# shuoshuof/Humanoid-Real-Time-Retarget

Measured on AMD Instinct MI355X. Metric: retargeted frames/sec + max joint-angle err vs ref, Hu humanoid @1/2/4/8 GPU, higher is better.
Workload: dtype f32; 1 GPU; VtrdynFullBodyPosRetargeter batched solve, Hu v5 target (BASELINE config 3); global_batch=262144, parallelism=dp1, input_layout=soa, input_ring_sets=3, precise_gripper=True, launch=K plain launches, step i on stream i % 2

## Files before the change

__graft_entry__.py:

```python
from __future__ import annotations

import os
import shutil
import subprocess
import sys

REPO = os.path.dirname(os.path.abspath(__file__))
PKG = os.path.join(REPO, "humanoid-real-time-retarget_amd")
ORACLE = os.path.join(REPO, "oracle")
for _p in (PKG, ORACLE):
    if _p not in sys.path:
        sys.path.insert(0, _p)


def _jobs() -> str:
    return str(min(16, os.cpu_count() or 1))


CSRC = os.path.join(PKG, "csrc")
FASTMATH_SRC = os.path.join(REPO, "tools", "check_fastmath.hip")
FASTMATH_BIN = os.path.join(REPO, "tools", "check_fastmath")
FDIV_SRC = os.path.join(REPO, "tools", "check_fdiv.hip")
FDIV_BIN = os.path.join(REPO, "tools", "check_fdiv")
FETCH_CALIB_BIN = os.path.join(REPO, "tools", "fetch_calib")


def _make(*args, env=None) -> None:
    env = dict(os.environ if env is None else env)
    env.setdefault("HIPCC", shutil.which("hipcc") or "/opt/rocm/bin/hipcc")
    subprocess.run(["make", "-C", CSRC, *args], check=True, env=env)


def build_fastmath_check(env=None) -> str:
    _make("check_fastmath", env=env)
    return FASTMATH_BIN


def build_fdiv_check(env=None) -> str:
    _make("check_fdiv", env=env)
    return FDIV_BIN


def build_fetch_calib(env=None) -> str:
    _make("fetch_calib", env=env)
    return FETCH_CALIB_BIN


def build() -> None:
    env = dict(os.environ)
    env.setdefault("HIPCC", shutil.which("hipcc") or "/opt/rocm/bin/hipcc")
    _make("-j", _jobs(), "all", "variants", env=env)
    subprocess.run(["make", "-C", ORACLE], check=True, env=env)
    build_fastmath_check(env)
    build_fdiv_check(env)
    build_fetch_calib(env)
    from rtg.build_ext import build_frame_post
    build_frame_post()
    import rtg
    from rtg import _lib
    _lib.lib()


def smoke() -> None:
    import numpy as np
    import torch

    import oracle as orc
    from rtg import _lib, assets
    from rtg.runtime import Solver

    assert torch.cuda.is_available(), "smoke() needs a HIP device"
    g = np.load(os.path.join(REPO, "tests", "golden", "full_body_pos_precise.npz"))
    zp = np.load(os.path.join(REPO, "tests", "golden", "zero_pose.npz"))
    n = 256
    body, lh, rh = (np.ascontiguousarray(g[k][:n]) for k in ("body", "lh", "rh"))
    S = Solver(_lib.SOLVER_FULL_BODY_POS, zp["vtrdyn_full_local_t"], zp["vtrdyn_full_global_t"],
               assets.parents("vtrdyn_full"), precise_gripper=True)
    dof, _, _ = S.retarget([torch.from_numpy(a).cuda() for a in (body, lh, rh)])
    torch.cuda.synchronize()
    dof = dof.cpu().numpy()
    odof, _, _ = orc.full_body_pos(zp["vtrdyn_full_local_t"], zp["vtrdyn_full_global_t"], body, lh, rh, True,
                                   want_rot=False)
    diff_oracle = float(np.abs(dof - odof).max())
    diff_ref = float(np.abs(dof - g["dof"][:n]).max())
    exact = float(np.mean(dof == odof))
    e = np.load(os.path.join(REPO, "tests", "golden", "full_body_pos_edge.npz"))
    edof, _, _ = S.retarget([torch.from_numpy(np.ascontiguousarray(e[k])).cuda() for k in ("body", "lh", "rh")])
    edof = edof.cpu().numpy()
    eodof, _, _ = orc.full_body_pos(zp["vtrdyn_full_local_t"], zp["vtrdyn_full_global_t"], e["body"], e["lh"], e["rh"],
                                    True, want_rot=False)
    status = orc.frame_status(edof)
    print(f"smoke: {n} frames; max|gpu-oracle|={diff_oracle:.3g} (exact {exact:.4f}); "
          f"max|gpu-reference|={diff_ref:.3g}; {len(edof)} degenerate frames, {int((status > 0).sum())} marked where "
          f"the reference raises ({int((e['precise_status'] > 0).sum())})")
    assert np.isfinite(dof).all()
    np.testing.assert_array_equal(dof, odof, err_msg="GPU path disagrees with the oracle (bit for bit)")
    def bits(a):
        return np.where(np.isnan(a), np.uint32(0x7FC00000), a.view(np.uint32))
    np.testing.assert_array_equal(bits(edof), bits(eodof),
                                  err_msg="GPU path disagrees with the oracle on degenerate frames (bit for bit)")
    np.testing.assert_array_equal(status, e["precise_status"], err_msg="frames marked != frames the reference raised on")
    assert diff_ref <= 2.13e-5, "GPU path outside the measured reference residual"


if __name__ == "__main__":
    build()
    if len(sys.argv) > 1 and sys.argv[1] == "smoke":
        smoke()
```

humanoid-real-time-retarget_amd/csrc/rtg_knobs.h:

```cpp
#pragma once

#ifndef RTG_SIDES_TILES
#define RTG_SIDES_TILES 2
#endif
#ifndef RTG_SIDES_EARLY_WORDS
#define RTG_SIDES_EARLY_WORDS 1
#endif
#ifndef RTG_AOS_PRELOAD_TIPS
#define RTG_AOS_PRELOAD_TIPS 1
#endif
#ifndef RTG_SIDES_SOA_WAVES
#define RTG_SIDES_SOA_WAVES 5
#endif
#ifndef RTG_SIDES_UNIFORM_WAVE
#define RTG_SIDES_UNIFORM_WAVE 3
#endif
#ifndef RTG_QUAD8_MAX_B
#define RTG_QUAD8_MAX_B 2048
#endif
#ifndef RTG_QUAD_MAX_B
#define RTG_QUAD_MAX_B 4096
#endif
#ifndef RTG_LATENCY_MAX_B
#define RTG_LATENCY_MAX_B 49152
#endif
#ifndef RTG_EXP_HOT_INPUTS
#define RTG_EXP_HOT_INPUTS 0
#endif
#ifndef RTG_EXP_TIMESTAMPS
#define RTG_EXP_TIMESTAMPS 0
#endif
#ifndef RTG_EXP_SKIP_SIGNAL
#define RTG_EXP_SKIP_SIGNAL 0
#endif
#ifndef RTG_VEL_SEG
#define RTG_VEL_SEG 10
#endif
#ifndef RTG_VEL_LDS_MIN
#define RTG_VEL_LDS_MIN 0
#endif
#ifndef RTG_FK_NT_OUT
#define RTG_FK_NT_OUT 1
#endif
#ifndef RTG_FK_F16_MAXJ
#define RTG_FK_F16_MAXJ 36
#endif
#ifndef RTG_EXP_MULR_NOBRANCH
#define RTG_EXP_MULR_NOBRANCH 0
#endif
#ifndef RTG_EXP_NO_TABLE
#define RTG_EXP_NO_TABLE 0
#endif
#ifndef RTG_TORSO_X0
#define RTG_TORSO_X0 1
#endif
#ifndef RTG_FIT_FAST_DIV
#define RTG_FIT_FAST_DIV 1
#endif
#ifndef RTG_FIT_FAST_DIV_TU
#define RTG_FIT_FAST_DIV_TU RTG_FIT_FAST_DIV
#endif
#ifndef RTG_DOF_NT_STORE
#define RTG_DOF_NT_STORE 1
#endif
#ifndef RTG_VEL_W
#define RTG_VEL_W 8
#endif
#ifndef RTG_DOF_NWAY
#define RTG_DOF_NWAY 4
#endif
#ifndef RTG_UNIT_TAB_K
#define RTG_UNIT_TAB_K 16
#endif
#ifndef RTG_SIDES_SHARED_FIT
#define RTG_SIDES_SHARED_FIT 1
#endif
#ifndef RTG_EULER_LIBM
#define RTG_EULER_LIBM 1
#endif
#ifndef RTG_UPPER_UNIT_TAB
#define RTG_UPPER_UNIT_TAB 1
#endif
#ifndef RTG_ROT_UNIT_TAB
#define RTG_ROT_UNIT_TAB 1
#endif
#ifndef RTG_SIDES_UNIT_TAB
#define RTG_SIDES_UNIT_TAB 7
#endif
#ifndef RTG_SIDES_UNIT_TAB_AOS
#define RTG_SIDES_UNIT_TAB_AOS 1
#endif
#ifndef RTG_FRAME1_UNIT_TAB
#define RTG_FRAME1_UNIT_TAB 6
#endif
#ifndef RTG_FK_UNIT_TAB
#define RTG_FK_UNIT_TAB 1
#endif
#ifndef RTG_DOF_UNIT_TAB
#define RTG_DOF_UNIT_TAB 1
#endif
#ifndef RTG_VEL_UNIT_TAB
#define RTG_VEL_UNIT_TAB 1
#endif
#ifndef RTG_VEL_ANG_NB
#define RTG_VEL_ANG_NB 2
#endif
#ifndef RTG_ROT_INGEST_TILE_AOS
#define RTG_ROT_INGEST_TILE_AOS 16
#endif
#ifndef RTG_ROT_INGEST_TILE_SOA
#define RTG_ROT_INGEST_TILE_SOA 16
#endif
#ifndef RTG_EXP_NO_RARE
#define RTG_EXP_NO_RARE 0
#endif
#ifndef RTG_EXP_STUB_SVD
#define RTG_EXP_STUB_SVD 0
#endif
```

humanoid-real-time-retarget_amd/csrc/rtg_math.cuh:

```cuda
#pragma once
#include <hip/hip_runtime.h>
#include <stdint.h>

#include "rtg_crmath.h"
#include "rtg_knobs.h"

#pragma clang fp contract(off)

namespace rtg {

struct Q { float x, y, z, w; };
struct V { float x, y, z; };

#define RTG_DEV __device__ __forceinline__

RTG_DEV float ieee_sqrtf(float x) { return __builtin_sqrtf(x); }
RTG_DEV float cr_sqrt(float x)
{
    const bool tiny = x < 0x1p-96f;
    const float xs = tiny ? x * 0x1p64f : x;
    float s = __builtin_amdgcn_sqrtf(xs);
    const float sdn = __uint_as_float(__float_as_uint(s) - 1u), sup = __uint_as_float(__float_as_uint(s) + 1u);
    const float rdn = __builtin_fmaf(-sdn, s, xs), rup = __builtin_fmaf(-sup, s, xs);
    s = rdn <= 0.0f ? sdn : s;
// ... 474 lines not shown
#pragma unroll
        for (int i = 0; i < N; ++i)
            if (!ok[i]) out[i] = qnormalize(q0[i]);
    }
}
struct NoTab {};
template <int N>
RTG_DEV void qnormalize_n_t(const Q (&q)[N], Q (&out)[N], NoTab) { qnormalize_n<N>(q, out); }
template <int N>
RTG_DEV void qnormalize_n_t(const Q (&q)[N], Q (&out)[N], const UnitEnt *tab) { qnormalize_tab_n<N>(q, tab, out); }
RTG_DEV Q qnormalize_t(Q q, NoTab) { return qnormalize(q); }
template <typename Tab>
RTG_DEV Q qfrom_angle_unit_axis_t(float angle, V axis, Tab tab)
{
    const float theta = angle / 2.0f;
    const SC t = cr_sincos((double)theta);
    return qnormalize_t(Q{axis.x * t.s, axis.y * t.s, axis.z * t.s, t.c}, tab);
}
template <bool ON> struct TabSel {
    static RTG_DEV const UnitEnt *get(const UnitEnt *t) { return t; }
};
template <> struct TabSel<false> {
    static RTG_DEV NoTab get(const UnitEnt *) { return NoTab{}; }
};
RTG_DEV Q qnormalize_t(Q q, const UnitEnt *tab)
{
    const Q a[1] = {q};
    Q o[1];
    qnormalize_tab_n<1>(a, tab, o);
    return o[0];
}

template <int N, typename Tab = NoTab>
RTG_DEV void qfrom_angle_unit_axis_n(const float (&angle)[N], const V (&axis)[N], Q (&out)[N], Tab tab = Tab{})
{
    double th[N];
#pragma unroll
    for (int i = 0; i < N; ++i) th[i] = (double)(angle[i] / 2.0f);
    SC t[N];
    cr_sincos_n<N>(th, t);
    Q q[N];
#pragma unroll
    for (int i = 0; i < N; ++i) q[i] = Q{axis[i].x * t[i].s, axis[i].y * t[i].s, axis[i].z * t[i].s, t[i].c};
    qnormalize_n_t<N>(q, out, tab);
}

template <typename Tab = NoTab>
RTG_DEV Q qfrom_rotmat(const float m[9], Tab tab = Tab{})
{
    const float d0 = m[0], d1 = m[4], d2 = m[8];
    float w = cr_sqrt(clamp_lo((((d0 + d1) + d2) + 1.0f) / 4.0f, 0.0f));
    float x = cr_sqrt(clamp_lo((((d0 - d1) - d2) + 1.0f) / 4.0f, 0.0f));
    float y = cr_sqrt(clamp_lo((((-d0 + d1) - d2) + 1.0f) / 4.0f, 0.0f));
    float z = cr_sqrt(clamp_lo((((-d0 - d1) + d2) + 1.0f) / 4.0f, 0.0f));
    if (w >= x && w >= y && w >= z) {
        x *= tsign(m[7] - m[5]);
        y *= tsign(m[2] - m[6]);
        z *= tsign(m[3] - m[1]);
    }
    if (x >= w && x >= y && x >= z) {
        w *= tsign(m[7] - m[5]);
        y *= tsign(m[3] + m[1]);
        z *= tsign(m[2] + m[6]);
    }
    if (y >= w && y >= x && y >= z) {
        w *= tsign(m[2] - m[6]);
        x *= tsign(m[3] + m[1]);
        z *= tsign(m[7] + m[5]);
    }
    if (z >= w && z >= x && z >= y) {
        w *= tsign(m[3] - m[1]);
        x *= tsign(m[6] + m[2]);
        y *= tsign(m[7] + m[5]);
    }
    return qnormalize_t(Q{x, y, z, w}, tab);
}

RTG_DEV V qexp_map(Q q)
{
    const float sin_theta = cr_sqrt(1.0f - q.w * q.w);
    float angle = 2.0f * cr_acos(q.w);
    angle = normalize_angle(angle);
    const bool mask = fabsf(sin_theta) > 1e-5f;
    const float a = mask ? angle : 0.0f;
    const float ax = mask ? q.x / sin_theta : 0.0f;
    const float ay = mask ? q.y / sin_theta : 0.0f;
    const float az = mask ? q.z / sin_theta : 1.0f;
    return V{a * ax, a * ay, a * az};
}
RTG_DEV Q qangle_axis(Q q)
{
    const float sin_theta = cr_sqrt(1.0f - q.w * q.w);
    float angle = 2.0f * cr_acos(q.w);
    angle = normalize_angle(angle);
    const bool mask = fabsf(sin_theta) > 1e-5f;
    const Rcp r = rcp64(sin_theta);
    const V u = mulr_v(V{q.x, q.y, q.z}, r);
    return Q{mask ? angle : 0.0f, mask ? u.x : 0.0f, mask ? u.y : 0.0f, mask ? u.z : 1.0f};
}
RTG_DEV float qexp_component(Q q, int k)
{
    const V e = qexp_map(q);
    return k == 0 ? e.x : (k == 1 ? e.y : e.z);
}

constexpr uint32_t kAngTabLo = 0x3e800000u;
constexpr uint32_t kAngTabEntries = 0x3f800000u - kAngTabLo;
constexpr uint32_t kAngTabBits = 3;
constexpr uint32_t kAngTabPer = 10u;
constexpr uint32_t kAngTabWords = (kAngTabEntries + kAngTabPer - 1) / kAngTabPer;
constexpr uint32_t kAngTabBias = 1u << (kAngTabBits - 1);
RTG_DEV uint32_t ang_tab_word(uint32_t i) { return __umulhi(i, 0xCCCCCCCDu) >> 3; }
RTG_DEV float exp_angle_estimate(float w)
{
    const float t2 = (1.0f - w) * 0.5f;
    const float t = __builtin_amdgcn_sqrtf(t2);
    float p = __builtin_fmaf(0.04965998747593211f, t2, -0.005969297163659217f);
    p = __builtin_fmaf(p, t2, 0.029188122223620813f);
    p = __builtin_fmaf(p, t2, 0.02938421651028137f);
    p = __builtin_fmaf(p, t2, 0.0447135443846629f);
    p = __builtin_fmaf(p, t2, 0.07499796602478857f);
    p = __builtin_fmaf(p, t2, 0.1666666806527845f);
    return 4.0f * __builtin_fmaf(t, t2 * p, t);
}
RTG_DEV uint32_t ang_tab_code(float w)
{
    const float R = normalize_angle(2.0f * cr_acos(w));
    const float P = exp_angle_estimate(w);
    if (!(R > 0.0f) || !(P > 0.0f) || !(R < 4.0f) || !(P < 4.0f)) return 0u;
    const int32_t d = (int32_t)__float_as_uint(R) - (int32_t)__float_as_uint(P);
    const int32_t lim = (int32_t)kAngTabBias - 1;
    return (d >= -lim && d <= lim) ? (uint32_t)(d + (int32_t)kAngTabBias) : 0u;
}
RTG_DEV uint32_t ang_tab_build_word(uint32_t wd)
{
    uint32_t word = 0;
    for (uint32_t e = 0; e < kAngTabPer; ++e) {
        const uint32_t i = wd * kAngTabPer + e;
        if (i < kAngTabEntries) word |= ang_tab_code(__uint_as_float(kAngTabLo + i)) << (kAngTabBits * e);
    }
    return word;
}
RTG_DEV float exp_dof_tab(float w, float qk, const uint32_t *__restrict__ tab)
{
    const uint32_t i = __float_as_uint(w) - kAngTabLo;
    const bool in = i < kAngTabEntries;
#if RTG_EXP_NO_TABLE
    const uint32_t wd = ang_tab_word(i);
    const uint32_t word = 0x24924924u + 0u * tab[0];
#else
    const uint32_t wd = ang_tab_word(i);
    const uint32_t word = tab[in ? wd : 0u];
#endif
    const float sin_theta = cr_sqrt(1.0f - w * w);
    const bool mask = fabsf(sin_theta) > 1e-5f;
    const float P = exp_angle_estimate(w);
    const uint32_t code = in ? (word >> ((i - wd * kAngTabPer) * kAngTabBits)) & ((1u << kAngTabBits) - 1u) : 0u;
    float angle = __uint_as_float(__float_as_uint(P) + code - kAngTabBias);
    if (__builtin_expect(mask && code == 0u, 0)) angle = normalize_angle(2.0f * cr_acos(w));
    return mask ? angle * (qk / sin_theta) : 0.0f;
}
struct ExpDof {
    float angle, sin_theta;
    bool mask, exact;
};
RTG_DEV uint32_t ang_tab_word_of(float w)
{
    const uint32_t i = __float_as_uint(w) - kAngTabLo;
    return i < kAngTabEntries ? ang_tab_word(i) : 0u;
}
RTG_DEV ExpDof exp_dof_word_part(float w, uint32_t word);
RTG_DEV ExpDof exp_dof_table_part(float w, const uint32_t *__restrict__ tab)
{
#if RTG_EXP_NO_TABLE
    const uint32_t word = 0x24924924u + 0u * tab[0];
#else
    const uint32_t word = tab[ang_tab_word_of(w)];
#endif
    return exp_dof_word_part(w, word);
}
RTG_DEV ExpDof exp_dof_word_part(float w, uint32_t word)
{
    const uint32_t i = __float_as_uint(w) - kAngTabLo;
    const bool in = i < kAngTabEntries;
    const uint32_t wd = ang_tab_word(i);
#if RTG_EXP_NO_TABLE
    word = 0x24924924u;
#endif
    const float sin_theta = cr_sqrt(1.0f - w * w);
    const bool mask = fabsf(sin_theta) > 1e-5f;
    const float P = exp_angle_estimate(w);
    const uint32_t code = in ? (word >> ((i - wd * kAngTabPer) * kAngTabBits)) & ((1u << kAngTabBits) - 1u) : 0u;
    return ExpDof{__uint_as_float(__float_as_uint(P) + code - kAngTabBias), sin_theta, mask, mask && code == 0u};
}
RTG_DEV float exp_dof_finish(const ExpDof &e, float qk) { return e.mask ? e.angle * (qk / e.sin_theta) : 0.0f; }
__device__ __attribute__((noinline)) float exp_dof_exact(float w, float qk)
{
    const float angle = normalize_angle(2.0f * cr_acos(w));
    return angle * (qk / cr_sqrt(1.0f - w * w));
}
RTG_DEV float qexp_component_tab(Q q, int k, const uint32_t *__restrict__ tab)
{
    return exp_dof_tab(q.w, k == 0 ? q.x : (k == 1 ? q.y : q.z), tab);
}

RTG_DEV float dot3(V a, V b) { return (a.x * b.x + a.y * b.y) + a.z * b.z; }
RTG_DEV float lnorm3(V a)
{
    return cr_sqrt(__builtin_fmaf(a.z, a.z, __builtin_fmaf(a.y, a.y, a.x * a.x)));
}
RTG_DEV V cross3(V a, V b)
{
    return V{__builtin_fmaf(a.y, b.z, -(a.z * b.y)), __builtin_fmaf(a.z, b.x, -(a.x * b.z)),
             __builtin_fmaf(a.x, b.y, -(a.y * b.x))};
}
RTG_DEV V vsub(V a, V b) { return V{a.x - b.x, a.y - b.y, a.z - b.z}; }
RTG_DEV V vdiv(V a, float s)
{
    const Rcp r = rcp64(s);
    return mulr_v(a, r);
}
RTG_DEV V vmul(V a, float s) { return V{s * a.x, s * a.y, s * a.z}; }
RTG_DEV V vunit(V a)
{
    const Rcp r = sqrt_clamp_rcp(__builtin_fmaf(a.z, a.z, __builtin_fmaf(a.y, a.y, a.x * a.x)), 0.0f).r;
    return mulr_v(a, r);
}

RTG_DEV V proj_in_plane(V v, V n)
{
    const float nn = lnorm3(n);
    return vsub(v, vmul(n, dot3(v, n) / (nn * nn)));
}

RTG_DEV float radians_between(V v1, V v2, V n);
RTG_DEV float radians_between_axes(V v1, V v2, V n)
{
    v2 = vunit(v2);
    const float c = clamp_lohi(dot3(v1, v2), -1.0f, 1.0f);
    return cr_acos(c) * tsign(dot3(n, cross3(v1, v2)));
}


RTG_DEV Q exp_map_angle_axis(V e)
{
    const NormRcp nr = sqrt_clamp_rcp(__builtin_fmaf(e.z, e.z, __builtin_fmaf(e.y, e.y, e.x * e.x)), 0.0f);
    const float n = nr.n;
    const Rcp r = nr.r;
    const float a = normalize_angle(n);
    const bool mask = fabsf(a) > 1e-5f;
    const V u = mulr_v(e, r);
    return Q{mask ? a : 0.0f, mask ? u.x : 0.0f, mask ? u.y : 0.0f, mask ? u.z : 1.0f};
}
RTG_DEV Q qslerp(Q q0, Q q1, float t)
{
    float ch = ((q0.x * q1.x + q0.y * q1.y) + q0.z * q1.z) + q0.w * q1.w;
    if (ch < 0.0f) q1 = Q{-q1.x, -q1.y, -q1.z, -q1.w};
    ch = fabsf(ch);
    const float half = cr_acos(ch);
    const float sh = cr_sqrt(1.0f - ch * ch);
    const float ra = cr_sin((1.0f - t) * half) / sh;
    const float rb = cr_sin(t * half) / sh;
    if (fabsf(ch) >= 1.0f) return q0;
    if (fabsf(sh) < 0.001f)
        return Q{0.5f * q0.x + 0.5f * q1.x, 0.5f * q0.y + 0.5f * q1.y, 0.5f * q0.z + 0.5f * q1.z, 0.5f * q0.w + 0.5f * q1.w};
    return Q{ra * q0.x + rb * q1.x, ra * q0.y + rb * q1.y, ra * q0.z + rb * q1.z, ra * q0.w + rb * q1.w};
}
RTG_DEV float rotmat_det(const float m[9])
{
    const float t1 = m[0] * (m[4] * m[8] - m[5] * m[7]);
    const float t2 = m[1] * (m[3] * m[8] - m[5] * m[6]);
    const float t3 = m[2] * (m[3] * m[7] - m[4] * m[6]);
    return (t1 - t2) + t3;
}
RTG_DEV void rotmat_from_quat(Q q, float o[9])
{
    const float i = q.x, j = q.y, k = q.z, r = q.w;
    const float two_s = 2.0f / (((i * i + j * j) + k * k) + r * r);
    o[0] = 1.0f - two_s * (j * j + k * k);
    o[1] = two_s * (i * j - k * r);
    o[2] = two_s * (i * k + j * r);
    o[3] = two_s * (i * j + k * r);
    o[4] = 1.0f - two_s * (i * i + k * k);
    o[5] = two_s * (j * k - i * r);
    o[6] = two_s * (i * k - j * r);
    o[7] = two_s * (j * k + i * r);
    o[8] = 1.0f - two_s * (i * i + j * j);
}
RTG_DEV float axis_angle_of(Q q, int axis)
{
    if (axis == 0) return g_atan2f(2.0f * (q.w * q.x + q.y * q.z), 1.0f - 2.0f * (q.x * q.x + q.z * q.z));
    if (axis == 1) return g_atan2f(2.0f * (q.w * q.y + q.x * q.z), 1.0f - 2.0f * (q.y * q.y + q.z * q.z));
    return g_atan2f(2.0f * (q.w * q.z + q.x * q.y), 1.0f - 2.0f * (q.z * q.z + q.y * q.y));
}
RTG_DEV Q axis_half_quat(int axis, float a)
{
    const float h = a / 2.0f;
    const float s = cr_sin(h), c = cr_cos(h);
    return Q{axis == 0 ? s : 0.0f, axis == 1 ? s : 0.0f, axis == 2 ? s : 0.0f, c};
}

RTG_DEV float fdiv(float a, float b)
{
    return a / b;
}
RTG_DEV float la_sqrt(float x)
{
    return cr_sqrt(x);
}
RTG_DEV float la_sqrt_nt(float x) { return cr_sqrt_nt(x); }
constexpr float kDivLo = 0x1p-47f, kDivHi = 0x1p47f;
RTG_DEV bool fdiv_in_window(float x)
{
    const float ax = fabsf(x);
    return (ax >= kDivLo) & (ax <= kDivHi);
}
template <int N>
RTG_DEV void fdiv_n_bare(const float (&a)[N], float b, float (&q)[N])
{
    float y = __builtin_amdgcn_rcpf(b);
    y = __builtin_fmaf(__builtin_fmaf(-b, y, 1.0f), y, y);
#pragma unroll
    for (int i = 0; i < N; ++i) {
        float t = a[i] * y;
        t = __builtin_fmaf(__builtin_fmaf(-b, t, a[i]), y, t);
        q[i] = __builtin_fmaf(__builtin_fmaf(-b, t, a[i]), y, t);
    }
}
template <int N>
RTG_DEV void fdiv_n(const float (&a)[N], float b, float (&q)[N])
{
#if RTG_FIT_FAST_DIV_TU
    bool ok = fdiv_in_window(b);
#pragma unroll
    for (int i = 0; i < N; ++i) ok &= fdiv_in_window(a[i]);
    fdiv_n_bare<N>(a, b, q);
    if (__builtin_expect(!ok, 0)) {
#pragma unroll
        for (int i = 0; i < N; ++i) q[i] = a[i] / b;
    }
#else
#pragma unroll
    for (int i = 0; i < N; ++i) q[i] = a[i] / b;
#endif
}
RTG_DEV float la_sign(float a, float b) { return __builtin_copysignf(fabsf(a), b); }
RTG_DEV float la_lapy2(float x, float y)
{
    const float xa = fabsf(x), ya = fabsf(y);
    const float w = fmaxf(xa, ya), z = fminf(xa, ya);
    const float r = fdiv(z, w);
    return z == 0.0f ? w : w * la_sqrt_nt(1.0f + r * r);
}
template <int NX>
RTG_DEV float la_larfg(float &alpha, float &x0, float &x1)
{
    const float safmin = 1.17549435e-38f / 5.96046448e-08f, rsafmn = 1.0f / safmin;
    float xn = NX == 1 ? fabsf(x0) : la_lapy2(x0, x1);
    float beta = -__builtin_copysignf(la_lapy2(alpha, xn), alpha);
    int knt = 0;
    if (__builtin_expect((xn == 0.0f) | (fabsf(beta) < safmin), 0)) {
        if (xn == 0.0f) return 0.0f;
        do {
            ++knt;
            x0 *= rsafmn;
            if (NX == 2) x1 *= rsafmn;
            beta *= rsafmn;
            alpha *= rsafmn;
        } while (fabsf(beta) < safmin && knt < 20);
        xn = NX == 1 ? fabsf(x0) : la_lapy2(x0, x1);
        beta = -__builtin_copysignf(la_lapy2(alpha, xn), alpha);
    }
    const float tau = fdiv(beta - alpha, beta);
    const float sc = fdiv(1.0f, alpha - beta);
    x0 *= sc;
    if (NX == 2) x1 *= sc;
    for (int j = 0; j < knt; ++j) beta *= safmin;
    alpha = beta;
    return tau;
}
RTG_DEV void la_lartg(float f, float g, float &c, float &s, float &r)
{
    const float safmin = 1.17549435e-38f, safmax = 1.0f / safmin;
    const float rtmin = 1.08420217e-19f, rtmax = 1.30438176e+19f;
    const float f1 = fabsf(f), g1 = fabsf(g);
#if RTG_FIT_FAST_DIV_TU
    const bool common = (f1 >= kDivLo) & (f1 <= kDivHi) & (g1 >= kDivLo) & (g1 <= kDivHi);
    {
        const float d = la_sqrt_nt(f * f + g * g);
        const float num[2] = {f1, g};
        float quo[2];
        fdiv_n_bare<2>(num, d, quo);
        c = quo[0];
        r = __builtin_copysignf(d, f);
        s = f < 0.0f ? -quo[1] : quo[1];
    }
#else
    const bool common = (g != 0.0f) & (f != 0.0f) & (f1 > rtmin) & (f1 < rtmax) & (g1 > rtmin) & (g1 < rtmax);
    {
        const float d = la_sqrt(f * f + g * g);
        const float quo[2] = {fdiv(f1, d), fdiv(g, d)};
        c = quo[0];
        r = __builtin_copysignf(d, f);
        s = f < 0.0f ? -quo[1] : quo[1];
    }
#endif
    if (__builtin_expect(!common, 0)) {
        if (g == 0.0f) { c = 1.0f; s = 0.0f; r = f; }
        else if (f == 0.0f) { c = 0.0f; s = __builtin_copysignf(1.0f, g); r = g1; }
#if RTG_FIT_FAST_DIV_TU
        else if ((f1 > rtmin) & (f1 < rtmax) & (g1 > rtmin) & (g1 < rtmax)) {
            const float d = la_sqrt(f * f + g * g), q = fdiv(g, d);
            c = fdiv(f1, d);
            r = __builtin_copysignf(d, f);
            s = f < 0.0f ? -q : q;
        }
#endif
        else {
            const float u = fminf(safmax, fmaxf(safmin, fmaxf(f1, g1)));
            const float fs = fdiv(f, u), gs = fdiv(g, u), d = la_sqrt(fs * fs + gs * gs);
            c = fdiv(fabsf(fs), d);
            r = __builtin_copysignf(d, f);
            s = fdiv(gs, r);
            r *= u;
        }
    }
}
RTG_DEV float la_las2_min(float f, float g, float h)
{
    const float fa = fabsf(f), ga = fabsf(g), ha = fabsf(h);
    const float fhmn = fminf(fa, ha), fhmx = fmaxf(fa, ha);
    if (fhmn == 0.0f) return 0.0f;
    if (ga < fhmx) {
        const float num[3] = {fhmn, fhmx - fhmn, ga};
        float quo[3];
        fdiv_n<3>(num, fhmx, quo);
        const float as = 1.0f + quo[0], at = quo[1];
        float au = quo[2];
        au = au * au;
        const float c = fdiv(2.0f, la_sqrt_nt(as * as + au) + la_sqrt(at * at + au));
        return fhmn * c;
    }
    const float au = fdiv(fhmx, ga);
    if (au == 0.0f) return fdiv(fhmn * fhmx, ga);
    const float num[2] = {fhmn, fhmx - fhmn};
    float quo[2];
    fdiv_n<2>(num, fhmx, quo);
    const float as = 1.0f + quo[0], at = quo[1], p = as * au, q = at * au;
    const float c = fdiv(1.0f, la_sqrt_nt(1.0f + p * p) + la_sqrt_nt(1.0f + q * q));
    const float mn = (fhmn * c) * au;
    return mn + mn;
}
RTG_DEV void la_lasv2(float f, float g, float h, float &ssmin, float &ssmax, float &snr, float &csr, float &snl,
                      float &csl)
{
    const float eps = 5.96046448e-08f;
    float ft = f, fa = fabsf(ft), ht = h, ha = fabsf(h), gt = g;
    float clt = 1.0f, crt = 1.0f, slt = 0.0f, srt = 0.0f;
    int pmax = 1;
    const bool swap = ha > fa;
    if (swap) { pmax = 3; float t = ft; ft = ht; ht = t; t = fa; fa = ha; ha = t; }
    const float ga = fabsf(gt);
    if (ga == 0.0f) { ssmin = ha; ssmax = fa; }
    else {
        bool gasmal = true;
        if (ga > fa) {
            pmax = 2;
            if (fdiv(fa, ga) < eps) {
                gasmal = false;
                ssmax = ga;
                ssmin = ha > 1.0f ? fdiv(fa, fdiv(ga, ha)) : fdiv(fa, ga) * ha;
                const float num[2] = {ht, ft};
                float quo[2];
                fdiv_n<2>(num, gt, quo);
                clt = 1.0f; slt = quo[0]; srt = 1.0f; crt = quo[1];
            }
        }
        if (gasmal) {
#if RTG_FIT_FAST_DIV_TU
// ... 864 lines not shown
```

humanoid-real-time-retarget_amd/csrc/rtg_ops.hip:

```cpp
#include "rtg_device.cuh"

namespace rtg {

struct Dir3 {
    float x, y, z;
    int32_t on;
};

__global__ __launch_bounds__(256) void k_rescale_motion(TopoView T, const float *__restrict__ motion, int64_t B,
                                                        Dir3 dir, float *__restrict__ out)
{
    const int64_t f = (int64_t)blockIdx.x * blockDim.x + threadIdx.x;
    if (f >= B) return;
    const int J = T.J;
    const float *m = motion + f * J * 3;
    float *o = out + f * J * 3;
    auto mp = [&](int j) {
        const V v = ld3(m + 3 * j);
        return dir.on ? V{v.x * dir.x, v.y * dir.y, v.z * dir.z} : v;
    };
    for (int j = 0; j < J; ++j) {
        const int p = ld_const(T.parents + j);
        const V mj = mp(j);
        if (p < 0) {
// ... 762 lines not shown
        for (int c = 0; c < 3; ++c) {
            lh[lay_idx(soa, f, i, c, 20, 3, B)] = jit(14 + i, c);
            rh[lay_idx(soa, f, i, c, 20, 3, B)] = jit(39 + i, c);
        }
    }
}

hipError_t launch_rescale_motion(const TopoView &T, const float *motion, int64_t B, const float *dir, float *out,
                                 hipStream_t s)
{
    const Dir3 d = dir ? Dir3{dir[0], dir[1], dir[2], 1} : Dir3{1.0f, 1.0f, 1.0f, 0};
    hipLaunchKernelGGL(k_rescale_motion, dim3(grid_for(B, 256)), dim3(256), 0, s, T, motion, B, d, out);
    return hipGetLastError();
}

hipError_t launch_quat_between(const float *v1, const float *v2, int64_t n, float *out, float *ws, hipStream_t s)
{
    hipError_t e = hipMemsetAsync(ws, 0, 2 * sizeof(float), s);
    if (e != hipSuccess) return e;
    hipLaunchKernelGGL(k_qbtv_norm_max, dim3(grid_for(n, 256)), dim3(256), 0, s, v1, v2, n, ws);
    hipLaunchKernelGGL(k_quat_between, dim3(grid_for(n, 256)), dim3(256), 0, s, v1, v2, n, ws, out);
    return hipGetLastError();
}

hipError_t launch_rebuild_vtrdyn(const TopoView &T, const float *motion, int64_t B, float *g_rot, float *root_t,
                                 float *ws, hipStream_t s)
{
    hipError_t e = hipMemsetAsync(ws, 0, T.J * sizeof(float), s);
    if (e != hipSuccess) return e;
    hipLaunchKernelGGL(k_rebuild_norm_max, dim3(grid_for(B, 256)), dim3(256), 0, s, T, motion, B, ws);
    hipLaunchKernelGGL(k_rebuild_vtrdyn, dim3(grid_for(B, 256)), dim3(256), 0, s, T, motion, B, ws, g_rot, root_t);
    return hipGetLastError();
}

hipError_t launch_ingest_vtrdyn(const float *bp, const float *lhp, const float *rhp, int64_t B, int layout,
                                float *body, float *lh, float *rh, uint8_t *valid, hipStream_t s)
{
    if (layout == RTG_LAYOUT_SOA)
        hipLaunchKernelGGL(k_ingest_vtrdyn<kIngSoaTile>, dim3(grid_for(B, kIngSoaTile)), dim3(256), 0, s, bp,
                           lhp, rhp, B, body, lh, rh, valid, true);
    else
        hipLaunchKernelGGL(k_ingest_vtrdyn<kIngAosTile>, dim3(grid_for(B, kIngAosTile)), dim3(256), 0, s, bp,
                           lhp, rhp, B, body, lh, rh, valid, false);
    return hipGetLastError();
}

hipError_t launch_quat_op(int op, const float *a, const float *b, const float *c, int64_t n, float *out,
                          hipStream_t s)
{
    hipLaunchKernelGGL(k_quat_op, dim3(grid_for(n, 256)), dim3(256), 0, s, op, a, b, c, n, out);
    return hipGetLastError();
}

hipError_t launch_cal_joint_quat(const float *Z, const float *M, int npts, int64_t n, float *out, hipStream_t s)
{
    const dim3 g(grid_for(n, 256)), b(256);
    switch (npts) {
    case 1: hipLaunchKernelGGL(k_cal_joint_quat<1>, g, b, 0, s, Z, M, n, out); break;
    case 2: hipLaunchKernelGGL(k_cal_joint_quat<2>, g, b, 0, s, Z, M, n, out); break;
    case 3: hipLaunchKernelGGL(k_cal_joint_quat<3>, g, b, 0, s, Z, M, n, out); break;
    case 4: hipLaunchKernelGGL(k_cal_joint_quat<4>, g, b, 0, s, Z, M, n, out); break;
    case 5: hipLaunchKernelGGL(k_cal_joint_quat<5>, g, b, 0, s, Z, M, n, out); break;
    case 6: hipLaunchKernelGGL(k_cal_joint_quat<6>, g, b, 0, s, Z, M, n, out); break;
    case 7: hipLaunchKernelGGL(k_cal_joint_quat<7>, g, b, 0, s, Z, M, n, out); break;
    default: hipLaunchKernelGGL(k_cal_joint_quat<8>, g, b, 0, s, Z, M, n, out); break;
    }
    return hipGetLastError();
}

hipError_t launch_quat_as_euler(const float *q, int s0, int s1, int s2, int extrinsic, int degrees, int64_t n,
                               double *out, hipStream_t s)
{
    hipLaunchKernelGGL(k_quat_as_euler, dim3(grid_for(n, 256)), dim3(256), 0, s, q, s0, s1, s2, extrinsic, degrees, n,
                       out);
    return hipGetLastError();
}
hipError_t launch_quat_in_xyz_axis(const float *q, int s0, int s1, int s2, int extrinsic, int64_t n, float *out,
                                   hipStream_t s)
{
    hipLaunchKernelGGL(k_quat_in_xyz_axis, dim3(grid_for(n, 256)), dim3(256), 0, s, q, s0, s1, s2, extrinsic, n, out);
    return hipGetLastError();
}

hipError_t launch_synth_full_body(const TopoView &T, uint64_t seed, int64_t off, int64_t B, float *body, float *lh,
                                  float *rh, float *body_rot, int layout, hipStream_t s)
{
    hipLaunchKernelGGL(k_synth_full_body, dim3(grid_for(B, 64)), dim3(64), 0, s, T, seed, off, B, body, lh, rh,
                       body_rot,
                       layout == RTG_LAYOUT_SOA);
    return hipGetLastError();
}

constexpr int kProbeIters = 4096;
__global__ __launch_bounds__(256) void k_probe_valu(float seed, float *__restrict__ sink, uint64_t *__restrict__ clk)
{
    float a[8];
#pragma unroll
    for (int k = 0; k < 8; ++k) a[k] = seed + (float)(threadIdx.x + k);
    const bool rec = (blockIdx.x & 63) == 0 && threadIdx.x == 0;
    uint64_t c0 = 0, w0 = 0;
    if (rec) {
        c0 = clock64();
        w0 = wall_clock64();
    }
    for (int i = 0; i < kProbeIters; ++i) {
#pragma unroll
        for (int k = 0; k < 8; ++k) a[k] = __builtin_fmaf(a[k], 0.999999f, 1e-7f);
    }
    if (rec) {
        const uint64_t c1 = clock64(), w1 = wall_clock64();
        clk[2 * (blockIdx.x >> 6)] = c1 - c0;
        clk[2 * (blockIdx.x >> 6) + 1] = w1 - w0;
    }
    float s = 0.0f;
#pragma unroll
    for (int k = 0; k < 8; ++k) s += a[k];
    if (s == 12345.678f) sink[threadIdx.x] = s;
}
__global__ __launch_bounds__(256) void k_probe_copy(const float4 *__restrict__ src, float4 *__restrict__ dst,
                                                    int64_t n)
{
    for (int64_t i = (int64_t)blockIdx.x * 256 + threadIdx.x; i < n; i += (int64_t)gridDim.x * 256) dst[i] = src[i];
}

hipError_t launch_probe_valu(int nblocks, float *sink, uint64_t *clk, hipStream_t s)
{
    hipLaunchKernelGGL(k_probe_valu, dim3(nblocks), dim3(256), 0, s, 1.0f, sink, clk);
    return hipGetLastError();
}
hipError_t launch_probe_copy(const float *src, float *dst, int64_t nfloat4, hipStream_t s)
{
    hipLaunchKernelGGL(k_probe_copy, dim3(256 * 32), dim3(256), 0, s, reinterpret_cast<const float4 *>(src),
                       reinterpret_cast<float4 *>(dst), nfloat4);
    return hipGetLastError();
}
int probe_valu_iters() { return kProbeIters; }

}

#if RTG_EXP_STUB_SVD + RTG_EXP_NO_TABLE + RTG_EXP_HOT_INPUTS + RTG_EXP_MULR_NOBRANCH + RTG_EXP_NO_RARE + \
    RTG_EXP_TIMESTAMPS + RTG_EXP_SKIP_SIGNAL == 0
#define RTG_WRONG_ANSWER_KNOBS 0
#else
#define RTG_WRONG_ANSWER_KNOBS 1
#endif
#define RTG_STR2(x) #x
#define RTG_STR(x) RTG_STR2(x)
#define RTG_KNOB(k) "\"" #k "\":\"" RTG_STR(k) "\","
extern "C" const char *rtg_build_info(void)
{
    return "{\"abi\":" RTG_STR(RTG_ABI_VERSION) ",\"arch\":\"gfx950\",\"knobs\":{"
        RTG_KNOB(RTG_DOF_NWAY) RTG_KNOB(RTG_DOF_UNIT_TAB) RTG_KNOB(RTG_FK_UNIT_TAB) RTG_KNOB(RTG_UNIT_TAB_K) RTG_KNOB(RTG_SIDES_SHARED_FIT) RTG_KNOB(RTG_UPPER_UNIT_TAB) RTG_KNOB(RTG_ROT_UNIT_TAB) RTG_KNOB(RTG_EULER_LIBM) RTG_KNOB(RTG_SIDES_UNIT_TAB) RTG_KNOB(RTG_SIDES_UNIT_TAB_AOS) RTG_KNOB(RTG_FRAME1_UNIT_TAB) RTG_KNOB(RTG_VEL_UNIT_TAB) RTG_KNOB(RTG_SIDES_SOA_WAVES) RTG_KNOB(RTG_SIDES_UNIFORM_WAVE) RTG_KNOB(RTG_SIDES_TILES) RTG_KNOB(RTG_SIDES_EARLY_WORDS) RTG_KNOB(RTG_AOS_PRELOAD_TIPS) RTG_KNOB(RTG_QUAD8_MAX_B) RTG_KNOB(RTG_QUAD_MAX_B) RTG_KNOB(RTG_LATENCY_MAX_B)
        RTG_KNOB(RTG_EXP_TIMESTAMPS) RTG_KNOB(RTG_EXP_SKIP_SIGNAL) RTG_KNOB(RTG_EXP_STUB_SVD) RTG_KNOB(RTG_EXP_NO_TABLE) RTG_KNOB(RTG_EXP_MULR_NOBRANCH) RTG_KNOB(RTG_FK_F16_MAXJ) RTG_KNOB(RTG_FK_NT_OUT) RTG_KNOB(RTG_TORSO_X0) RTG_KNOB(RTG_VEL_SEG) RTG_KNOB(RTG_VEL_LDS_MIN) RTG_KNOB(RTG_DOF_NT_STORE) RTG_KNOB(RTG_VEL_W) RTG_KNOB(RTG_VEL_ANG_NB) RTG_KNOB(RTG_EXP_NO_RARE)
        RTG_KNOB(RTG_ROT_INGEST_TILE_AOS) RTG_KNOB(RTG_ROT_INGEST_TILE_SOA) RTG_KNOB(RTG_FIT_FAST_DIV) RTG_KNOB(RTG_FIT_FAST_DIV_TU)
        "\"RTG_EXP_HOT_INPUTS\":\"" RTG_STR(RTG_EXP_HOT_INPUTS) "\"},\"wrong_answer_knobs\":"
        RTG_STR(RTG_WRONG_ANSWER_KNOBS) "}";
}
```

humanoid-real-time-retarget_amd/csrc/rtg_solver.cuh:

```cuda
#pragma once
#include "rtg_device.cuh"

namespace rtg {

struct Emit {
    float *row;
    float *__restrict__ lr;
    const uint32_t *__restrict__ ang;
    float2 *st;
    int sst;
    uint32_t *wd = nullptr;
    template <int LINK>
    static constexpr int slot() { return LINK <= 18 ? LINK - 12 : LINK - 14; }
    RTG_DEV void load_word(int s, float w) const
    {
#if !RTG_EXP_NO_TABLE
        __builtin_amdgcn_global_load_lds((const __attribute__((address_space(1))) void *)(ang + ang_tab_word_of(w)),
                                         (__attribute__((address_space(3))) void *)(wd + s * 64), 4, 0, 0);
#endif
    }
    template <int LINK>
    RTG_DEV void link(Q q) const
    {
        constexpr int k = hu_dof_axis(LINK - 1);
// ... 27 lines not shown
                    row[j < 7 ? 11 + j : 13 + j] = exp_dof_exact(v.x, v.y);
                }
        }
    }
    static RTG_DEV void wait_words() { __builtin_amdgcn_s_waitcnt(0x0F70); }
};

RTG_DEV void emit_fixed_links(const Emit &E, bool write_lr = true, int k0 = 0)
{
#pragma unroll
    for (int k = 0; k < 11; ++k)
        if (k >= k0) E.row[k] = 0.0f;
    E.row[29] = 0.0f;
    if (E.lr && write_lr) {
#pragma unroll
        for (int j = 0; j < 12; ++j) st4(E.lr + 4 * j, qident());
        st4(E.lr + 4 * 19, qident());
        st4(E.lr + 4 * 20, qident());
        st4(E.lr + 4 * 28, qident());
        st4(E.lr + 4 * 29, qident());
        st4(E.lr + 4 * 30, qident());
    }
}

enum : uint32_t {
    kStTorsoSvd = 1,
    kStLeftSvd = 2,
    kStLeftEuler = 4,
    kStRightSvd = 8,
    kStRightEuler = 16,
};
RTG_DEV uint32_t frame_error_code(uint32_t bits)
{
    const uint32_t first = bits & (0u - bits);
    return (first & (kStTorsoSvd | kStLeftSvd | kStRightSvd)) ? RTG_FRAME_SVD_NONFINITE : RTG_FRAME_ZERO_NORM_QUAT;
}
RTG_DEV void poison_frame(float *drow, float *__restrict__ lr, float *__restrict__ br, uint32_t bits)
{
    const float qn = __builtin_bit_cast(float, RTG_FRAME_NAN);
    drow[0] = __builtin_bit_cast(float, RTG_FRAME_NAN | frame_error_code(bits));
#pragma unroll
    for (int k = 1; k < 30; ++k) drow[k] = qn;
    const Q qq{qn, qn, qn, qn};
    if (lr)
        for (int j = 0; j < 31; ++j) st4(lr + 4 * j, qq);
    if (br)
        for (int j = 0; j < 59; ++j) st4(br + 4 * j, qq);
}

RTG_DEV void report_device_error(uint32_t *err, uint32_t code)
{
    if (err) __hip_atomic_fetch_or(err, code, __ATOMIC_RELAXED, __HIP_MEMORY_SCOPE_SYSTEM);
}

template <int L0, typename Tab = NoTab>
RTG_DEV Q solve_arm(const Emit &E, V upper, V fore, ArmZero zs, ArmZero ze, Q parent, Tab tab = Tab{})
{
    Q p, r, y, e;
    {
        const V v[1] = {upper};
        const ArmZero z[1] = {zs};
        const Q par[1] = {parent};
        Q a[1], b[1];
        arm_pair_n<true, 1>(v, z, par, a, b, tab);
        p = a[0];
        r = b[0];
    }
    E.link<L0>(p);
    E.link<L0 + 1>(r);
    {
        const V v[1] = {fore};
        const ArmZero z[1] = {ze};
        const Q par[1] = {qmul(qmul(parent, p), r)};
        Q a[1], b[1];
        arm_pair_n<false, 1>(v, z, par, a, b, tab);
        y = a[0];
        e = b[0];
    }
    E.link<L0 + 2>(y);
    E.link<L0 + 3>(e);
    return qmul(qmul(qmul(p, r), y), e);
}

RTG_DEV void link_rt(const Emit &E, int link, Q q)
{
    const int k = kHuDofAxis[link - 1];
    E.st[(link <= 18 ? link - 12 : link - 14) * E.sst] = make_float2(q.w, k == 0 ? q.x : (k == 1 ? q.y : q.z));
    if (E.lr) st4(E.lr + 4 * link, q);
}
template <int L0>
RTG_DEV bool emit_euler_xyz(const Emit &E, Q local)
{
    Q eul[3];
    const bool refused = quat_in_xyz_intrinsic(local, eul);
    E.link<L0>(eul[0]);
    E.link<L0 + 1>(eul[1]);
    E.link<L0 + 2>(eul[2]);
    return refused;
}

RTG_DEV float hand_x_mean(Q rot, V h0, const V (&tip)[5])
{
    const float x0 = qrotate(rot, h0).x;
    return mean5(qrotate(rot, tip[0]).x - x0, qrotate(rot, tip[1]).x - x0, qrotate(rot, tip[2]).x - x0,
                 qrotate(rot, tip[3]).x - x0, qrotate(rot, tip[4]).x - x0);
}
template <bool SOA>
struct FV;
template <>
struct FV<false> {
    const float *__restrict__ p;
    RTG_DEV V p3(int j) const { return ld3(p + 3 * j); }
    RTG_DEV Q q4(int j) const { return ld4(p + 4 * j); }
};
template <>
struct FV<true> {
    const float *__restrict__ p;
    int64_t s;
    RTG_DEV float e(int64_t i) const { return p[i]; }
    RTG_DEV V p3(int j) const { return V{e((3 * j) * s), e((3 * j + 1) * s), e((3 * j + 2) * s)}; }
    RTG_DEV Q q4(int j) const { return Q{e((4 * j) * s), e((4 * j + 1) * s), e((4 * j + 2) * s), e((4 * j + 3) * s)}; }
};
template <bool SOA>
RTG_DEV FV<SOA> frame_view(const float *__restrict__ base, int64_t f, int row_floats, int64_t B);
template <>
RTG_DEV FV<false> frame_view<false>(const float *__restrict__ base, int64_t f, int row_floats, int64_t)
{
    return FV<false>{base + f * row_floats};
}
template <>
RTG_DEV FV<true> frame_view<true>(const float *__restrict__ base, int64_t f, int, int64_t B)
{
    return FV<true>{base + f, B};
}

template <typename View>
RTG_DEV float hand_x_mean(Q rot, const View &H, const int (&idx)[5])
{
    const V tip[5] = {H.p3(idx[0]), H.p3(idx[1]), H.p3(idx[2]), H.p3(idx[3]), H.p3(idx[4])};
    return hand_x_mean(rot, H.p3(0), tip);
}

constexpr int kDofStride = 31;

RTG_DEV void store_dof_rows(float *__restrict__ dst, const float *src, int64_t nrows, int t, int nthr)
{
    const int nvals = (int)nrows * 30;
    auto at = [&](int i) {
        const int rr = i / 30;
        return src[rr * kDofStride + (i - rr * 30)];
    };
    const int nvec = nvals >> 2;
    typedef float f4v __attribute__((ext_vector_type(4)));
    for (int v = t; v < nvec; v += nthr) {
        const int i = v << 2;
        const f4v q = {at(i), at(i + 1), at(i + 2), at(i + 3)};
        if (RTG_DOF_NT_STORE) __builtin_nontemporal_store(q, reinterpret_cast<f4v *>(dst + i));
        else *reinterpret_cast<f4v *>(dst + i) = q;
    }
    for (int i = (nvec << 2) + t; i < nvals; i += nthr) dst[i] = at(i);
}

constexpr int kSideTiles = RTG_SIDES_TILES;
constexpr int kSideThreads = 128 * kSideTiles;
constexpr int kSideFrames = 64 * kSideTiles;

template <typename View, typename Hook = NoHook, typename Tab = NoTab>
RTG_DEV Q fbp_torso(const SolverConsts &C, const View &b, bool &svd_nan, const Hook &hook = Hook{}, Tab tab = Tab{})
{
    const V b10 = b.p3(10);
    const V Mt[3] = {vsub(b.p3(17), b10), vsub(b.p3(13), b10), vsub(b.p3(11), b10)};
    return cal_joint_quat<3>(C.Zt, Mt, svd_nan, hook, tab);
}
RTG_DEV Q upper_pt_sign(V v) { return Q{v.x * -1.0f, v.y * -1.0f, v.z * 1.0f, 0.0f}; }
template <typename View>
RTG_DEV Q upper_torso(const SolverConsts &C, const View &x, bool &svd_nan)
{
    auto pt = [&](int j) {
        const Q q = upper_pt_sign(x.p3(j));
        return V{q.x, q.y, q.z};
    };
    const V s10 = pt(10);
    const V Mt[3] = {vsub(pt(17), s10), vsub(pt(13), s10), vsub(pt(11), s10)};
    return cal_joint_quat<3>(C.Zt, Mt, svd_nan);
}
template <int SIDE, typename View, typename Hook = NoHook, typename Tab = NoTab>
RTG_DEV Q fbp_wrist_fit(const SolverConsts &C, const View &H, bool &svd_nan, const Hook &hook = Hook{}, Tab tab = Tab{})
{
    const V h0 = H.p3(0);
    const V M[5] = {vsub(H.p3(2), h0), vsub(H.p3(6), h0), vsub(H.p3(10), h0), vsub(H.p3(14), h0), vsub(H.p3(17), h0)};
    return cal_joint_quat<5>(SIDE ? C.Zr : C.Zl, M, svd_nan, hook, tab);
}
struct ArmPts { V sh, el, wr; };
struct TipPts { V h0, t[5]; };
template <int SIDE, typename View>
RTG_DEV ArmPts load_arm(const View &b)
{
    return ArmPts{b.p3(SIDE ? 14 : 18), b.p3(SIDE ? 15 : 19), b.p3(SIDE ? 16 : 20)};
}
template <typename View>
RTG_DEV TipPts load_tips(const View &H)
{
    return TipPts{H.p3(0), {H.p3(4), H.p3(8), H.p3(12), H.p3(16), H.p3(19)}};
}

template <typename Tab = NoTab>
RTG_DEV void fbp_arms2(const SolverConsts &C, const ArmPts &apL, const ArmPts &apR, Q R10, const Emit &E, Q &chL,
                       Q &chR, Tab tab = Tab{})
{
    const V up[2] = {vsub(apL.el, apL.sh), vsub(apR.el, apR.sh)};
    const V fo[2] = {vsub(apL.wr, apL.el), vsub(apR.wr, apR.el)};
    const ArmZero zs[2] = {C.lsh, C.rsh}, ze[2] = {C.lel, C.rel};
    const Q par[2] = {R10, R10};
    Q p[2], r[2], y[2], e[2];
    arm_pair_n<true, 2>(up, zs, par, p, r, tab);
    E.link<12>(p[0]);
    E.link<13>(r[0]);
    E.link<21>(p[1]);
    E.link<22>(r[1]);
    const Q par2[2] = {qmul(qmul(R10, p[0]), r[0]), qmul(qmul(R10, p[1]), r[1])};
    arm_pair_n<false, 2>(fo, ze, par2, y, e, tab);
    E.link<14>(y[0]);
    E.link<15>(e[0]);
    E.link<23>(y[1]);
    E.link<24>(e[1]);
    chL = qmul(qmul(qmul(p[0], r[0]), y[0]), e[0]);
    chR = qmul(qmul(qmul(p[1], r[1]), y[1]), e[1]);
}
template <bool PRECISE>
RTG_DEV void fbp_gripper(const SolverConsts &C, float a, float *row_d0)
{
    if (PRECISE) {
        const float sc = clamp_lohi(a / C.orig - 0.5f, 0.0f, 0.5f) / 0.5f;
        row_d0[0] = sc * 0.044f;
        row_d0[1] = sc * -0.044f;
    } else {
        const bool closed = a / C.orig < 0.7f;
        row_d0[0] = closed ? 0.0f : 0.044f;
        row_d0[1] = closed ? 0.0f : -0.044f;
    }
}
template <int SIDE>
RTG_DEV void fbp_body_rows(float *__restrict__ brow, Q R10, Q W, bool const_rows = true)
{
    st4(brow + 4 * (SIDE ? 39 : 14), W);
    if (!SIDE) {
        if (const_rows) {
            for (int j = 0; j < 59; ++j)
                if (j != 14 && j != 39) st4(brow + 4 * j, j == 10 ? R10 : qident());
        } else {
            st4(brow + 4 * 10, R10);
        }
    }
}
template <bool PRECISE, int SIDE, typename Tab = NoTab>
RTG_DEV bool fbp_side_after_arm(const SolverConsts &C, const TipPts &tp, Q R10, Q chain, Q W, const Emit &E,
                                float *__restrict__ brow, Tab tab = Tab{})
{
    constexpr int E0 = SIDE ? 25 : 16, D0 = SIDE ? 27 : 18;
    const bool refused = emit_euler_xyz<E0>(E, qnormalize_t(qmul(qconj(qnormalize_t(qmul(R10, chain), tab)), W), tab));
    fbp_gripper<PRECISE>(C, hand_x_mean(qconj(W), tp.h0, tp.t), E.row + D0);
    if (brow) fbp_body_rows<SIDE>(brow, R10, W);
    return refused;
}

template <int SIDE, typename View, typename Tab = NoTab>
RTG_DEV void solve_upper_side(const SolverConsts &C, const View &x, Q R10, const Emit &E, Tab tab = Tab{})
{
    auto pt = [&](int j) {
        const Q q = upper_pt_sign(x.p3(j));
        return V{q.x, q.y, q.z};
    };
    constexpr int L0 = SIDE ? 21 : 12, E0 = SIDE ? 25 : 16, D0 = SIDE ? 27 : 18;
    constexpr int SH = SIDE ? 14 : 18, EL = SIDE ? 15 : 19, WR = SIDE ? 16 : 20;
    const V sel = pt(EL);
    solve_arm<L0>(E, vsub(sel, pt(SH)), vsub(pt(WR), sel), SIDE ? C.rsh : C.lsh, SIDE ? C.rel : C.lel, R10, tab);
    E.identity<E0>(); E.identity<E0 + 1>(); E.identity<E0 + 2>();
    E.row[D0] = 0.0f; E.row[D0 + 1] = 0.0f;
}

template <int SIDE, typename View, typename Tab = NoTab>
RTG_DEV bool solve_full_body_rot_side(const SolverConsts &C, const View &q, const View &b, const View &H,
                                      const Emit &E, Tab tab = Tab{})
{
    constexpr int L0 = SIDE ? 21 : 12, E0 = SIDE ? 25 : 16, D0 = SIDE ? 27 : 18;
    constexpr int SH = SIDE ? 14 : 18, EL = SIDE ? 15 : 19, WR = SIDE ? 16 : 20, PAR = SIDE ? 13 : 17;
    const Q par = q.q4(PAR);
    const V bel = b.p3(EL);
    const Q chain = solve_arm<L0>(E, vsub(bel, b.p3(SH)), vsub(b.p3(WR), bel), SIDE ? C.rsh : C.lsh,
                                  SIDE ? C.rel : C.lel, par, tab);
    const Q w = q.q4(WR);
    const bool refused = emit_euler_xyz<E0>(E, qnormalize_t(qmul(qconj(qnormalize_t(qmul(par, chain), tab)), w), tab));
    constexpr int tips[5] = {3, 7, 11, 15, 19};
    const bool closed = hand_x_mean(w, H, tips) / C.orig < 0.7f;
    E.row[D0] = closed ? 0.0f : 0.044f;
    E.row[D0 + 1] = closed ? 0.0f : -0.044f;
    return refused;
}

template <int SIDE, typename View, typename Tab = NoTab>
RTG_DEV bool solve_body_rot_side(const SolverConsts &C, const View &g, const Emit &E, Tab tab = Tab{})
{
    auto local = [&](int j, int p) { return qnormalize_t(qmul(qconj(g.q4(p)), g.q4(j)), tab); };
    constexpr int SH = SIDE ? 14 : 18, EL = SIDE ? 15 : 19, D0 = SIDE ? 27 : 18;
    Q s3[3], e3[3];
    bool refused = quat_in_xyz_axis(local(SH, C.par[SIDE ? 1 : 0]), 1, 0, 2, false, s3);
    refused |= quat_in_xyz_axis(local(EL, C.par[SIDE ? 3 : 2]), 2, 1, 0, false, e3);
    if (SIDE) {
        E.link<21>(s3[0]); E.link<22>(s3[1]); E.link<23>(qnormalize_t(qmul(e3[0], s3[2]), tab));
        E.link<24>(e3[1]); E.link<25>(e3[2]);
        E.identity<26>(); E.identity<27>();
// ... 900 lines not shown
```

Before: 4.378 billion frames/s.

## Strength-reduce dof row packing, use non-temporal sqrt in exp paths, parametrize fdiv corrections

The vectorised dof-row store loop now tracks row and column incrementally instead of dividing by 30 for each element, and handles the one-slot skip at column 28 with a single wrap offset. The exp-map sin_theta and exact-dof paths switch from cr_sqrt to cr_sqrt_nt. The fast-division Newton correction count becomes a knob, defaulting to one step instead of the previous two, with a new fdiv1 checker added to the build. Dropping a correction and changing the sqrt variant remove arithmetic but put bit-exactness against the oracle at risk.

```diff
diff --git a/__graft_entry__.py b/__graft_entry__.py
--- a/__graft_entry__.py
+++ b/__graft_entry__.py
@@ -22,6 +22,8 @@
 FASTMATH_BIN = os.path.join(REPO, "tools", "check_fastmath")
 FDIV_SRC = os.path.join(REPO, "tools", "check_fdiv.hip")
 FDIV_BIN = os.path.join(REPO, "tools", "check_fdiv")
+FDIV1_SRC = os.path.join(REPO, "tools", "check_fdiv1.hip")
+FDIV1_BIN = os.path.join(REPO, "tools", "check_fdiv1")
 FETCH_CALIB_BIN = os.path.join(REPO, "tools", "fetch_calib")
 
 
@@ -41,6 +43,11 @@
     return FDIV_BIN
 
 
+def build_fdiv1_check(env=None) -> str:
+    _make("check_fdiv1", env=env)
+    return FDIV1_BIN
+
+
 def build_fetch_calib(env=None) -> str:
     _make("fetch_calib", env=env)
     return FETCH_CALIB_BIN
@@ -53,6 +60,7 @@
     subprocess.run(["make", "-C", ORACLE], check=True, env=env)
     build_fastmath_check(env)
     build_fdiv_check(env)
+    build_fdiv1_check(env)
     build_fetch_calib(env)
     from rtg.build_ext import build_frame_post
     build_frame_post()
diff --git a/humanoid-real-time-retarget_amd/csrc/rtg_knobs.h b/humanoid-real-time-retarget_amd/csrc/rtg_knobs.h
--- a/humanoid-real-time-retarget_amd/csrc/rtg_knobs.h
+++ b/humanoid-real-time-retarget_amd/csrc/rtg_knobs.h
@@ -60,6 +60,12 @@
 #ifndef RTG_FIT_FAST_DIV_TU
 #define RTG_FIT_FAST_DIV_TU RTG_FIT_FAST_DIV
 #endif
+#ifndef RTG_FDIV_CORRECTIONS
+#define RTG_FDIV_CORRECTIONS 1
+#endif
+#if RTG_FDIV_CORRECTIONS != 1 && RTG_FDIV_CORRECTIONS != 2
+#error "RTG_FDIV_CORRECTIONS: 1 or 2 (fewer gives wrong quotients)"
+#endif
 #ifndef RTG_DOF_NT_STORE
 #define RTG_DOF_NT_STORE 1
 #endif
diff --git a/humanoid-real-time-retarget_amd/csrc/rtg_math.cuh b/humanoid-real-time-retarget_amd/csrc/rtg_math.cuh
--- a/humanoid-real-time-retarget_amd/csrc/rtg_math.cuh
+++ b/humanoid-real-time-retarget_amd/csrc/rtg_math.cuh
@@ -650,7 +650,7 @@
     const uint32_t wd = ang_tab_word(i);
     const uint32_t word = tab[in ? wd : 0u];
 #endif
-    const float sin_theta = cr_sqrt(1.0f - w * w);
+    const float sin_theta = cr_sqrt_nt(1.0f - w * w);
     const bool mask = fabsf(sin_theta) > 1e-5f;
     const float P = exp_angle_estimate(w);
     const uint32_t code = in ? (word >> ((i - wd * kAngTabPer) * kAngTabBits)) & ((1u << kAngTabBits) - 1u) : 0u;
@@ -685,7 +685,7 @@
 #if RTG_EXP_NO_TABLE
     word = 0x24924924u;
 #endif
-    const float sin_theta = cr_sqrt(1.0f - w * w);
+    const float sin_theta = cr_sqrt_nt(1.0f - w * w);
     const bool mask = fabsf(sin_theta) > 1e-5f;
     const float P = exp_angle_estimate(w);
     const uint32_t code = in ? (word >> ((i - wd * kAngTabPer) * kAngTabBits)) & ((1u << kAngTabBits) - 1u) : 0u;
@@ -695,7 +695,7 @@
 __device__ __attribute__((noinline)) float exp_dof_exact(float w, float qk)
 {
     const float angle = normalize_angle(2.0f * cr_acos(w));
-    return angle * (qk / cr_sqrt(1.0f - w * w));
+    return angle * (qk / cr_sqrt_nt(1.0f - w * w));
 }
 RTG_DEV float qexp_component_tab(Q q, int k, const uint32_t *__restrict__ tab)
 {
@@ -821,8 +821,9 @@
 #pragma unroll
     for (int i = 0; i < N; ++i) {
         float t = a[i] * y;
-        t = __builtin_fmaf(__builtin_fmaf(-b, t, a[i]), y, t);
-        q[i] = __builtin_fmaf(__builtin_fmaf(-b, t, a[i]), y, t);
+#pragma unroll
+        for (int k = 0; k < RTG_FDIV_CORRECTIONS; ++k) t = __builtin_fmaf(__builtin_fmaf(-b, t, a[i]), y, t);
+        q[i] = t;
     }
 }
 template <int N>
diff --git a/humanoid-real-time-retarget_amd/csrc/rtg_ops.hip b/humanoid-real-time-retarget_amd/csrc/rtg_ops.hip
--- a/humanoid-real-time-retarget_amd/csrc/rtg_ops.hip
+++ b/humanoid-real-time-retarget_amd/csrc/rtg_ops.hip
@@ -938,7 +938,7 @@
     return "{\"abi\":" RTG_STR(RTG_ABI_VERSION) ",\"arch\":\"gfx950\",\"knobs\":{"
         RTG_KNOB(RTG_DOF_NWAY) RTG_KNOB(RTG_DOF_UNIT_TAB) RTG_KNOB(RTG_FK_UNIT_TAB) RTG_KNOB(RTG_UNIT_TAB_K) RTG_KNOB(RTG_SIDES_SHARED_FIT) RTG_KNOB(RTG_UPPER_UNIT_TAB) RTG_KNOB(RTG_ROT_UNIT_TAB) RTG_KNOB(RTG_EULER_LIBM) RTG_KNOB(RTG_SIDES_UNIT_TAB) RTG_KNOB(RTG_SIDES_UNIT_TAB_AOS) RTG_KNOB(RTG_FRAME1_UNIT_TAB) RTG_KNOB(RTG_VEL_UNIT_TAB) RTG_KNOB(RTG_SIDES_SOA_WAVES) RTG_KNOB(RTG_SIDES_UNIFORM_WAVE) RTG_KNOB(RTG_SIDES_TILES) RTG_KNOB(RTG_SIDES_EARLY_WORDS) RTG_KNOB(RTG_AOS_PRELOAD_TIPS) RTG_KNOB(RTG_QUAD8_MAX_B) RTG_KNOB(RTG_QUAD_MAX_B) RTG_KNOB(RTG_LATENCY_MAX_B)
         RTG_KNOB(RTG_EXP_TIMESTAMPS) RTG_KNOB(RTG_EXP_SKIP_SIGNAL) RTG_KNOB(RTG_EXP_STUB_SVD) RTG_KNOB(RTG_EXP_NO_TABLE) RTG_KNOB(RTG_EXP_MULR_NOBRANCH) RTG_KNOB(RTG_FK_F16_MAXJ) RTG_KNOB(RTG_FK_NT_OUT) RTG_KNOB(RTG_TORSO_X0) RTG_KNOB(RTG_VEL_SEG) RTG_KNOB(RTG_VEL_LDS_MIN) RTG_KNOB(RTG_DOF_NT_STORE) RTG_KNOB(RTG_VEL_W) RTG_KNOB(RTG_VEL_ANG_NB) RTG_KNOB(RTG_EXP_NO_RARE)
-        RTG_KNOB(RTG_ROT_INGEST_TILE_AOS) RTG_KNOB(RTG_ROT_INGEST_TILE_SOA) RTG_KNOB(RTG_FIT_FAST_DIV) RTG_KNOB(RTG_FIT_FAST_DIV_TU)
+        RTG_KNOB(RTG_ROT_INGEST_TILE_AOS) RTG_KNOB(RTG_ROT_INGEST_TILE_SOA) RTG_KNOB(RTG_FIT_FAST_DIV) RTG_KNOB(RTG_FIT_FAST_DIV_TU) RTG_KNOB(RTG_FDIV_CORRECTIONS)
         "\"RTG_EXP_HOT_INPUTS\":\"" RTG_STR(RTG_EXP_HOT_INPUTS) "\"},\"wrong_answer_knobs\":"
         RTG_STR(RTG_WRONG_ANSWER_KNOBS) "}";
 }
diff --git a/humanoid-real-time-retarget_amd/csrc/rtg_solver.cuh b/humanoid-real-time-retarget_amd/csrc/rtg_solver.cuh
--- a/humanoid-real-time-retarget_amd/csrc/rtg_solver.cuh
+++ b/humanoid-real-time-retarget_amd/csrc/rtg_solver.cuh
@@ -203,11 +203,18 @@
     };
     const int nvec = nvals >> 2;
     typedef float f4v __attribute__((ext_vector_type(4)));
+    const int dr = (4 * nthr) / 30, dc = (4 * nthr) - dr * 30;
+    int rr = (4 * t) / 30, c = 4 * t - rr * 30;
     for (int v = t; v < nvec; v += nthr) {
         const int i = v << 2;
-        const f4v q = {at(i), at(i + 1), at(i + 2), at(i + 3)};
+        const float *p = src + rr * kDofStride + c;
+        const int wrap = c == 28 ? 1 : 0;
+        const f4v q = {p[0], p[1], p[2 + wrap], p[3 + wrap]};
         if (RTG_DOF_NT_STORE) __builtin_nontemporal_store(q, reinterpret_cast<f4v *>(dst + i));
         else *reinterpret_cast<f4v *>(dst + i) = q;
+        c += dc;
+        rr += dr;
+        if (c >= 30) { c -= 30; ++rr; }
     }
     for (int i = (nvec << 2) + t; i < nvals; i += nthr) dst[i] = at(i);
 }
```

Result: faster. 4.443 billion frames/s, median of 6 (+1.5%).
